# INDA23PlusPlus/isaklm-raytracer

Measured on AMD Instinct MI355X. Metric: Msamples/sec (W×H×spp/s) at 1920×1080; achieved HBM GB/s vs peak, higher is better.
Workload: dtype f32

## Files before the change

### include/isaklm_rt.h

```cpp
#ifndef ISAKLM_RT_H
#define ISAKLM_RT_H

#include <stddef.h>
#include <stdint.h>
#ifndef __cplusplus
#include <stdbool.h>
#endif

#ifdef __cplusplus
extern "C" {
#endif

#define RT_ABI_VERSION 12

typedef struct RtUChar4 { uint8_t x, y, z, w; } RtUChar4;

#ifdef ISAKLM_RT_CALLER_TYPES
#ifndef __cplusplus
#error "ISAKLM_RT_CALLER_TYPES: the reference's types are C++ (anonymous unions, constructors)"
#endif
struct Vec2D;
struct Vec3D;
struct Texture;
struct Material;
// ... 210 lines not shown
    int max_depth;
    int kernel;
    void *stream;
    unsigned long long *counters_device;
    unsigned long long *wave_times_device;
    int wf_tail;
    int wf_finish_waves;
    int profile;
    int wf_descent_cap;
    int wf_postpone;
    int wf_wide;
    int shard_id;
    int num_shards;
    int wf_pipelines;
    int wf_long_depth;
    int traversal;
    int overlap;
    int check_interval;
    int debug;
    int coalesce_passes;
} RtOptions;

#define RT_TRAVERSAL_BOUNDED 0
#define RT_TRAVERSAL_KD 1
#define RT_TRAVERSAL_BOUNDED_COUNTED 2
#define RT_DEBUG_CALL_LOG 1
#define RT_DEBUG_LONG_LOG 2
#define RT_DEBUG_CHECK_FAULT 4
#define RT_DEBUG_LONG_QUIT 8
#define RT_DEBUG_SERIAL_LONG_FIRST 16
#define RT_DEBUG_SERIAL_FIN_FIRST 32
#define RT_DEBUG_WIDE_CAP1 64
#define RT_DEBUG_COUNT_LONG_ONLY 128

typedef struct RtProfile {
    int iterations;
    int trace_launches, shade_launches, finish_launches;
    float start_ms;
    float trace_ms;
    float shade_ms;
    float finish_ms;
    float call_ms;
    float trace_union_ms;
    int pipelines;
} RtProfile;
int rt_last_profile(RtProfile *out);
int rt_profile_history(RtProfile *out, int cap, int *count, int reset);

#define RT_DEV_HIST_BINS 18
typedef struct RtDeviations {
    unsigned long long watchdog_paths;
    unsigned long long cut_paths;
    unsigned long long max_deep_depth;
    unsigned long long deep_paths;
    unsigned long long deep_hist[RT_DEV_HIST_BINS];
    unsigned long long bounded_checked;
    unsigned long long bounded_mismatches;
    float mismatch_ray[6];
    unsigned long long owed_pixels;
    unsigned long long owed_passes;
    unsigned long long long_safety_quits;
    unsigned long long stranded_pixels;
    unsigned long long check_dropped;
    unsigned long long linger_expiries;
    unsigned long long long_closed;
    unsigned long long wide_overflows;
// ... 136 lines not shown
```

### isaklm-raytracer_amd/csrc/bvh_trace.h

```cpp
#pragma once
#include "bvh_common.h"
#include "rt_kernels.h"

namespace rtk {

#if defined(__HIP_DEVICE_COMPILE__)
#define RT_CONST __attribute__((address_space(4)))
#else
#define RT_CONST
#endif
__device__ __forceinline__ RtF4 ldc4(const RtF4 *p)
{
    const RT_CONST RtF4 *q = (const RT_CONST RtF4 *)p;
    return RtF4{q->x, q->y, q->z, q->w};
}
__device__ __forceinline__ uint2 ldc_u2(const void *p)
{
    const RT_CONST uint32_t *q = (const RT_CONST uint32_t *)p;
    return make_uint2(q[0], q[1]);
}
__device__ __forceinline__ float ldc_f(const uint32_t *p) { return __uint_as_float(*(const RT_CONST uint32_t *)p); }
__device__ __forceinline__ uint4 ldc_u4(const uint32_t *p)
{
    const RT_CONST uint4 *q = (const RT_CONST uint4 *)p;
// ... 138 lines not shown
    if (!rt_bvh_box(lx.x, ly.x, lz.x, hx.x, hy.x, hz.x, sl, best, t0)) t0 = INFINITY;
    if (!rt_bvh_box(lx.y, ly.y, lz.y, hx.y, hy.y, hz.y, sl, best, t1)) t1 = INFINITY;
    if (!rt_bvh_box(lx.z, ly.z, lz.z, hx.z, hy.z, hz.z, sl, best, t2)) t2 = INFINITY;
    if (!rt_bvh_box(lx.w, ly.w, lz.w, hx.w, hy.w, hz.w, sl, best, t3)) t3 = INFINITY;
    auto cswap = [](float &ta, uint32_t &ra, float &tb, uint32_t &rb) {
        const bool sw = tb < ta;
        const float t = sw ? tb : ta, u = sw ? ta : tb;
        const uint32_t r = sw ? rb : ra, q = sw ? ra : rb;
        ta = t;
        tb = u;
        ra = r;
        rb = q;
    };
    cswap(t0, r0, t1, r1);
    cswap(t2, r2, t3, r3);
    cswap(t0, r0, t2, r2);
    cswap(t1, r1, t3, r3);
    cswap(t1, r1, t2, r2);
    if (t3 != INFINITY) {
        stk.put(sp, r3, t3);
        ++sp;
    }
    if (t2 != INFINITY) {
        stk.put(sp, r2, t2);
        ++sp;
    }
    if (t1 != INFINITY) {
        stk.put(sp, r1, t1);
        ++sp;
    }
    return t0 != INFINITY ? r0 : RT_BVH_EMPTY;
}

template <bool COUNT, bool PARK, typename STACK>
__device__ __forceinline__ bool bvh4_query(const RtDevScene &sc, Vec3D o, Vec3D d, float best0, STACK &stk, Cnt &cn,
                                           int cap, bool resume, BvhPark &pk)
{
    const RtSlab sl = rt_slab(o, d, rt_ray_margin(o.x, o.y, o.z, sc.bvh_scale));
    int sp = 0;
    uint32_t cur = 0;
    float best = best0;
    int tk = -1;
    if (PARK && resume) {
        sp = pk.sp;
        cur = pk.cur;
        best = pk.best;
        tk = pk.tk;
    }
    int steps = 0;
    while (true) {
        while (!(cur & RT_BVH_LEAF)) {
            if (PARK) {
                if (steps >= cap) {
                    pk.cur = cur;
                    pk.sp = sp;
                    pk.best = best;
                    pk.tk = tk;
                    return false;
                }
                ++steps;
            }
            if (COUNT) cn.v[RT_CNT_B_BVH_NODE]++;
            const uint32_t next = bvh4_children(sc, cur, sl, best, stk, sp);
            cur = next != RT_BVH_EMPTY ? next : bvh_pop(stk, sp, best);
        }
        if (cur == RT_BVH_EMPTY) break;
        const uint32_t first = (cur & ~RT_BVH_LEAF) >> 3, end = first + (cur & 7u) + 1u;
        if (COUNT) cn.v[RT_CNT_B_BVH_TRI] += end - first;
        leaf_scan_min<COUNT>(sc.bvh_a, sc.bvh_bary, first, end, o, d, best, tk, cn);
        cur = bvh_pop(stk, sp, best);
        if (cur == RT_BVH_EMPTY) break;
    }
    pk.best = best;
    pk.tk = tk;
    return true;
}

template <bool COUNT, typename STACK>
__device__ __forceinline__ float bvh4_bound(const RtDevScene &sc, Vec3D o, Vec3D d, float best, STACK &stk, Cnt &cn,
                                            int &tstar, int &tk)
{
    BvhPark pk;
    (void)bvh4_query<COUNT, false>(sc, o, d, best, stk, cn, 0, false, pk);
    tk = pk.tk;
    tstar = pk.tk >= 0 ? (int)sc.bvh_bary[pk.tk].tri : -1;
    return pk.best;
}
template <bool COUNT, typename STACK>
__device__ __forceinline__ float bvh4_bound(const RtDevScene &sc, Vec3D o, Vec3D d, float best, STACK &stk, Cnt &cn,
                                            int &tstar)
{
    int tk;
    return bvh4_bound<COUNT>(sc, o, d, best, stk, cn, tstar, tk);
}

template <bool COUNT>
__device__ __forceinline__ bool kd_certified(const RtDevScene &sc, const Vec3D o, const Vec3D d, const float entry,
                                             const float root_exit, const float s_min, const int tk, int &hit,
                                             float &hbx, float &hby, float &hbz, Cnt &c, const bool count = true)
{
#if RT_KD_CERT
    if (!sc.kd_cert.safe) return false;
    if (rt_kd_cert(sc.kd_cert, o, d, entry, root_exit, s_min, tk) != RT_CERT_OK) return false;
    const RtIsectBary *r = sc.bvh_bary + tk;
    float cx, cy, cz;
    if (!rt_tri_bary(ldc4(&r->b), ldc4(&r->c), ldc4(&r->d), ldc_f(&r->rd), o, d, s_min, cx, cy, cz))
        return false;
    if (COUNT && count) {
        c.v[RT_CNT_HIT]++;
        c.cert[0]++;
    }
    hit = (int)ldc_u2(&r->rd).y;
    hbx = cx;
    hby = cy;
    hbz = cz;
    return true;
// ... 69 lines not shown
        kd_pop(stk, sp, root_exit, node, entry, exit_);
    }
}

template <bool COUNT, typename STACK>
__device__ __forceinline__ int trace_bvh(const RtDevScene &sc, const Vec3D o, const Vec3D d, float &hbx, float &hby,
                                         float &hbz, STACK &stk, Cnt &c)
{
    if (COUNT) c.v[RT_CNT_RAY]++;
    float entry, exit_;
    if (!bbox_hit(sc, o, d, entry, exit_)) return -1;
    const float root_exit = exit_;
    float s_min = -INFINITY;
    int tstar = -1;
    if (rt_bounded_ray(o, d, sc.split_vals, sc.split_off)) {
        int tk = -1;
        s_min = RT_BVH4 ? bvh4_bound<COUNT>(sc, o, d, exit_, stk, c, tstar, tk)
                        : bvh_bound<COUNT>(sc, o, d, exit_, stk, c);
        if (!(s_min < root_exit)) return -1;
        int hit;
        if (kd_certified<COUNT>(sc, o, d, entry, root_exit, s_min, tk, hit, hbx, hby, hbz, c)) return hit;
    }
    float hs;
    const int h = kd_bounded<COUNT>(sc, o, d, entry, root_exit, s_min, tstar, hbx, hby, hbz, hs, stk, c);
    if (COUNT && h >= 0) c.cert[1]++;
    return h;
}

#define RT_PARK_DONE 0
#define RT_PARK_BVH 1
#define RT_PARK_KD 2
template <bool COUNT, typename STACK>
__device__ __forceinline__ int trace_bvh_park(const RtDevScene &sc, const Vec3D o, const Vec3D d, int &hit, float &hbx,
                                              float &hby, float &hbz, STACK &stk, Cnt &c, int cap, int resume,
                                              bool defer_kd, BvhPark &pk)
{
    if (COUNT && resume == RT_PARK_DONE) c.v[RT_CNT_RAY]++;
    hit = -1;
    float entry, exit_;
    if (!bbox_hit(sc, o, d, entry, exit_)) return RT_PARK_DONE;
    const float root_exit = exit_;
    float s_min = -INFINITY;
    int tstar = -1;
    if (rt_bounded_ray(o, d, sc.split_vals, sc.split_off)) {
        if (resume != RT_PARK_KD) {
            if (!bvh4_query<COUNT, true>(sc, o, d, exit_, stk, c, cap, resume == RT_PARK_BVH, pk)) return RT_PARK_BVH;
            if (!(pk.best < root_exit)) return RT_PARK_DONE;
            if (kd_certified<COUNT>(sc, o, d, entry, root_exit, pk.best, pk.tk, hit, hbx, hby, hbz, c))
                return RT_PARK_DONE;
            if (RT_KD_CERT && defer_kd) return RT_PARK_KD;
        }
        s_min = pk.best;
        if (pk.tk >= 0) tstar = (int)sc.bvh_bary[pk.tk].tri;
    }
    float hs;
    hit = kd_bounded<COUNT>(sc, o, d, entry, root_exit, s_min, tstar, hbx, hby, hbz, hs, stk, c);
    if (COUNT && hit >= 0) c.cert[1]++;
    return RT_PARK_DONE;
}

template <typename STACK>
__device__ __forceinline__ int trace_s(const RtDevScene &sc, const Vec3D o, const Vec3D d, float &hs, STACK &stk,
                                       Cnt &c)
{
    float entry, exit_;
    if (!bbox_hit(sc, o, d, entry, exit_)) return -1;
    float bx, by, bz;
    return kd_bounded<false, true>(sc, o, d, entry, exit_, -INFINITY, -1, bx, by, bz, hs, stk, c);
}

template <typename STACK>
__device__ __forceinline__ bool occluded_bvh(const RtDevScene &sc, const Vec3D o, const Vec3D d, const float tmax,
                                             STACK &stk, Cnt &c, bool &early)
{
    early = false;
    float entry, exit_;
    if (!bbox_hit(sc, o, d, entry, exit_)) return false;
    const float root_exit = exit_;
    const float best0 = fminf(root_exit, tmax);
// ... 14 lines not shown
```

### isaklm-raytracer_amd/csrc/host/trace_host.h

```cpp
#pragma once
#include <math.h>
#include <stdint.h>
#include <stdio.h>
#include <stdlib.h>
#include <string.h>

#include <algorithm>
#include <chrono>
#include <utility>
#include <vector>

#include "../bvh_common.h"
#include "bvh_build.h"
#include "rt_host.h"

namespace trace_host {

inline float bitsf(uint32_t u)
{
    float f;
    memcpy(&f, &u, 4);
    return f;
}
inline uint32_t fbits(float f)
// ... 221 lines not shown
            for (int k = 3; k >= 1; --k)
                if (t[k] != INFINITY) stk.push_back(B{r[k], t[k]});
            cur = t[0] != INFINITY ? r[0] : pop();
        }
        if (cur == RT_BVH_EMPTY) break;
        const uint32_t first = (cur & ~RT_BVH_LEAF) >> 3, end = first + (cur & 7u) + 1u;
        obs.bvh_leaf();
        for (uint32_t e = first; e < end; ++e) {
            float s, b[3];
            obs.bvh_test();
            if (!rt_tri_plane(h.bvh_a[e], o, d, INFINITY, s) || !(s <= best)) continue;
            const bool lt = s < best;
            if (!lt && tk < 0) continue;
            const RtIsectBary &R = h.bvh_bary[e];
            if (!rt_tri_bary(R.b, R.c, R.d, bitsf(R.rd), o, d, s, b[0], b[1], b[2])) continue;
            if (lt) {
                best = s;
                tk = (int)e;
            } else {
                tk = TK_TIE;
            }
        }
        cur = pop();
        if (cur == RT_BVH_EMPTY) break;
    }
    return Smin{best, tk};
}
inline Smin bvh4_smin(const rt_host::PreparedHost &h, Vec3D o, Vec3D d, float best)
{
    NoObserver none;
    return bvh4_smin(h, o, d, best, none);
}

template <class Obs>
float bvh_bound(const rt_host::PreparedHost &h, Vec3D o, Vec3D d, float best, Obs &obs)
{
    const RtSlab sl = rt_slab(o, d, rt_ray_margin(o.x, o.y, o.z, h.bvh_scale));
    struct B { uint32_t ref; float tn; };
    B stk[RT_BVH_STACK];
    int sp = 0;
    uint32_t cur = 0;
    while (true) {
        if (!(cur & RT_BVH_LEAF)) {
            obs.bvh_node();
            const RtF4 *nd = &h.bvh_nodes[4 * (size_t)cur];
            const uint32_t c0 = fbits(nd[3].x), c1 = fbits(nd[3].y);
            float tn0, tn1;
            const bool h0 = rt_bvh_box(nd[0].x, nd[0].y, nd[0].z, nd[0].w, nd[1].x, nd[1].y, sl, best, tn0) &&
                            c0 != RT_BVH_EMPTY;
            const bool h1 = rt_bvh_box(nd[1].z, nd[1].w, nd[2].x, nd[2].y, nd[2].z, nd[2].w, sl, best, tn1) &&
                            c1 != RT_BVH_EMPTY;
            if (h0 && h1) {
                const bool sf = tn1 < tn0;
                stk[sp++] = B{sf ? c0 : c1, sf ? tn0 : tn1};
                cur = sf ? c1 : c0;
                continue;
            }
            if (h0 || h1) {
                cur = h0 ? c0 : c1;
                continue;
            }
        } else {
            obs.bvh_leaf();
            const uint32_t first = (cur & ~RT_BVH_LEAF) >> 3, end = first + (cur & 7u) + 1u;
            for (uint32_t e = first; e < end; ++e) {
                float s, b[3];
// ... 288 lines not shown
```

### isaklm-raytracer_amd/csrc/wavefront.hip

```cpp
#include <hip/hip_runtime.h>

#include <stdio.h>
#include <stdlib.h>
#include <string.h>
#include <time.h>

#include <algorithm>
#include <chrono>
#include <atomic>
#include <map>
#include <mutex>
#include <thread>
#include <vector>

#include "bvh_trace.h"
#include "path_event.h"
#include "rt_kernels.h"
#include "rt_launch.h"
#include "rt_workspace.h"
#include "wf_check_grid.h"

using namespace rtk;

#include "wf_state.h"
// ... 443 lines not shown
    const RtDevFrame &fr = c.fr;
    const hipStream_t stream = c.stream;
    const int long_depth = c.long_depth, debug = c.debug;
    const uint32_t check_mask = c.check_mask;
    const size_t slots = (size_t)fr.width * fr.height;
    const bool chain_asked = c.overlap;
    const bool overlap = c.overlap && !fr.reset;
    if (!w.cus) {
        hipDeviceProp_t prop;
        w.cus = hipGetDeviceProperties(&prop, c.dev) == hipSuccess && prop.multiProcessorCount > 0
                    ? prop.multiProcessorCount
                    : 256;
    }
    const int grid = w.cus * 4 * WF_FIN_BVH_WAVES / (WF_BLOCK / 64);
    const ChainKey key = chain_key(c);
    const bool chained = overlap && w.chain_open && !fr.reset && memcmp(&key, &w.key, sizeof key) == 0;
    if (!chained && join_all(w, stream) != 0) return -1;
    if (ensure(w, slots, grid, 1) != 0) return -1;
    Pipe &pp = w.pipe[0];
    WfState st = pp.st;
    whole_state(st, c);
    const int long_return = st.long_return;
    st.fresh_n = (uint32_t)(((fr.width + 15) / 16) * ((fr.height + 15) / 16)) * 256u;
    st.linger = overlap ? 0ull : WF_FIN_LINGER;
    st.chk_mask = check_mask;
    const int par = (int)(w.call_seq & 1);
    unsigned long long chk_want = 0;
    if (ensure_records(w, wf_check_records(slots, (unsigned long long)fr.passes, check_mask,
                                           long_depth > 0 ? long_depth : RT_DEEP_PATH, WF_CHECK_CAP, &chk_want)) != 0)
        return -1;
    st.chk = check_mask == 0xFFFFFFFFu ? nullptr : w.chk + 3 * (size_t)w.chk_cap * (size_t)par;
    st.chk_cap = w.chk_cap;
    st.chk_ctr = w.chk_ctr + par;
    st.chk_fault = (debug & RT_DEBUG_CHECK_FAULT) ? 1 : 0;
    if ((debug & RT_DEBUG_LONG_LOG) && !w.long_log_buf &&
        hipMalloc((void **)&w.long_log_buf, 8 * 4 * 65536) != hipSuccess) {
        w.long_log_buf = nullptr;
        return -1;
    }
    unsigned long long *const long_log_buf = w.long_log_buf;
    st.long_log = (debug & RT_DEBUG_LONG_LOG) ? long_log_buf : nullptr;
    int fgrid = (int)((slots + WF_BLOCK - 1) / WF_BLOCK);
    const int fmax = long_return ? grid - WF_LONG_BLOCKS : grid;
    fgrid = fgrid > fmax ? fmax : fgrid;
    const uint32_t k = (uint32_t)(w.call_seq % 8);
    st.fin_live = long_return ? w.fin_live + k : nullptr;
    st.call_id = (uint32_t)w.call_seq + 1u;
    if (!chained) {
        if (long_return) {
            if (hipMemsetAsync(st.long_ctr, 0, 256, stream) != hipSuccess) return -1;
            if (hipMemsetAsync(st.long_ent, 0, (size_t)st.long_cap * 8, stream) != hipSuccess) return -1;
            if (hipMemsetAsync(st.ret_ring, 0, (size_t)st.long_cap * 8, stream) != hipSuccess) return -1;
            if (hipMemsetAsync(st.ret_ctr, 0, 256, stream) != hipSuccess) return -1;
        }
        if (st.long_log && hipMemsetAsync(long_log_buf, 0, 8 * 4 * 65536, stream) != hipSuccess) return -1;
    }
    ++w.call_seq;
    const hipStream_t s = pp.stream;
    if (hipEventRecord(w.fork, stream) != hipSuccess || hipStreamWaitEvent(s, w.fork, 0) != hipSuccess) return -1;
    if (hipMemsetAsync(st.counts, 0, 256, s) != hipSuccess) return -1;
    if (st.fin_live && hipMemsetD32Async((hipDeviceptr_t)st.fin_live, (int)(fgrid * (WF_BLOCK / 64)), 1, s) != hipSuccess)
        return -1;
    if (st.chk) {
        if (!w.chk_done[par].wait_on(s)) return -1;
        if (hipMemsetAsync(st.chk_ctr, 0, 4, s) != hipSuccess) return -1;
    }
    if (long_return && hipMemsetD32Async((hipDeviceptr_t)st.chain_flag, overlap ? 1 : 0, 1, s) != hipSuccess) return -1;
// ... 496 lines not shown
```

### isaklm-raytracer_amd/csrc/wf_finish_kernels.h

```cpp
#pragma once

namespace {

__device__ __forceinline__ uint32_t ld_sc1(const uint32_t *p)
{
    return __hip_atomic_load(const_cast<uint32_t *>(p), __ATOMIC_RELAXED, __HIP_MEMORY_SCOPE_AGENT);
}

__device__ __forceinline__ void st_sc1(uint32_t *p, uint32_t v)
{
    __hip_atomic_store(p, v, __ATOMIC_RELAXED, __HIP_MEMORY_SCOPE_AGENT);
}

__device__ __forceinline__ bool fresh_pixel(const RtDevFrame &fr, uint32_t e, int &slot)
{
    const uint32_t tiles_x = (uint32_t)(fr.width + 15) / 16u;
    const uint32_t t = e >> 8, w = (e >> 6) & 3u, l = e & 63u;
    const int x = (int)((t % tiles_x) * 16u + (w & 1u) * 8u + (l & 7u));
    const int y = (int)((t / tiles_x) * 16u + (w >> 1) * 8u + (l >> 3));
    if (x >= fr.width || y >= fr.height || !rt_row_owned(fr, y)) return false;
    slot = y * fr.width + x;
    return true;
}

// ... 25 lines not shown
    Cnt c;
    if (COUNT) c.zero();
    const uint32_t n_heavy = st.fresh && st.heavy_list ? *st.heavy_n : 0u;
    const uint32_t n = st.fresh ? n_heavy + st.fresh_n : st.counts[6 + q];
    const int limit = fr.max_depth > 0 ? fr.max_depth : RT_WATCHDOG_BOUNCES;
    const int lane = __lane_id();
    if (lane == 0) {
        unsigned long long *const ret_word = reinterpret_cast<unsigned long long *>(st.ret_ctr);
        if (st.fin_live && !(__hip_atomic_load(st.fin_live, __ATOMIC_RELAXED, __HIP_MEMORY_SCOPE_AGENT) & WF_FIN_STARTED))
            __hip_atomic_fetch_or(st.fin_live, WF_FIN_STARTED, __ATOMIC_RELAXED, __HIP_MEMORY_SCOPE_AGENT);
        if (st.long_return)
            __hip_atomic_fetch_add(ret_word, 1ull << 32, __ATOMIC_RELAXED, __HIP_MEMORY_SCOPE_AGENT);
        if (st.span) atomicMin(st.span, __builtin_amdgcn_s_memrealtime());
        if (st.long_log && blockIdx.x == 0 && threadIdx.x == 0) st.long_log[0] = __builtin_amdgcn_s_memrealtime();
    }
#if WF_NEE_LDS
    __shared__ float s_nee[10 * WF_BLOCK];
    PathRegsL p;
    p.rp.w = s_nee + wbase;
    p.cont.w = s_nee + 3 * WF_BLOCK + wbase;
    p.snorm.w = s_nee + 6 * WF_BLOCK + wbase;
    p.light.w = reinterpret_cast<int *>(s_nee + 9 * WF_BLOCK) + wbase;
#else
    PathRegs p;
#endif
    p.slot = 0;
    p.ro = p.rd = rt_v3(0, 0, 0);
    bool active = false, exhausted = false;
    bool rel = false;
    unsigned long long idle_since = 0;
    uint32_t quiet_trips = 0;
    uint32_t idle_trips = 0;
    bool seated = false;
#if WF_BVH_PARK
    __shared__ uint32_t s_pk_cur[WF_BLOCK];
    __shared__ int s_pk_sp[WF_BLOCK];
    __shared__ float s_pk_best[WF_BLOCK];
    __shared__ int s_pk_tk[WF_BLOCK];
    int parked = RT_PARK_DONE;
#endif
    while (true) {
        while (st.fresh && __any(rel)) {
            if (rel) {
                WfCold &cs = WF_COLD(st);
                uint32_t x = RT_PX_BUSY;
                if (__hip_atomic_compare_exchange_strong(cs.pxo + p.slot, &x, 0u, __ATOMIC_RELAXED, __ATOMIC_RELAXED,
                                                         __HIP_MEMORY_SCOPE_AGENT)) {
                    rel = false;
                } else {
                    x = __hip_atomic_exchange(cs.pxo + p.slot, RT_PX_BUSY, __ATOMIC_RELAXED, __HIP_MEMORY_SCOPE_AGENT);
                    const uint32_t owed = x & RT_PX_PASSES;
                    __hip_atomic_fetch_max(cs.ret_ctr + 5, owed, __ATOMIC_RELAXED, __HIP_MEMORY_SCOPE_AGENT);
                    __hip_atomic_fetch_add(cs.ret_ctr + 6, 1u, __ATOMIC_RELAXED, __HIP_MEMORY_SCOPE_AGENT);
                    const RtDevFrame cf = WF_COLD_FRAME(fr);
                    atomicAdd(cf.dev_stats + RT_DEV_OWED_PIXELS, 1ull);
                    atomicAdd(cf.dev_stats + RT_DEV_OWED_PASSES, (unsigned long long)owed);
                    p.passes_left = (int)owed;
                    const Vec3D fb = cf.fb[p.slot];
                    const float sq = cf.sq[p.slot];
                    const int count = cf.count[p.slot];
                    if (start_sample<COUNT>(cf, WF_COLD_CAM(cam), (int)p.slot, p.passes_left, p.rng, fb, sq, count, p.ro, p.rd,
                                            c)) {
                        begin_path(p);
                        rel = false;
                        active = true;
                    }
                }
            }
        }
        if (st.long_return) {
            const bool chained = st.linger == 0ull;
            const bool idle = !active && !(chained && exhausted);
            const unsigned long long im = __ballot(idle);
// ... 152 lines not shown
                if (idle_since == 0) idle_since = __builtin_amdgcn_s_memrealtime();
                if (__hip_atomic_load(cs.long_ctr + 3, __ATOMIC_RELAXED, __HIP_MEMORY_SCOPE_AGENT) == 0u)
                    ++quiet_trips;
                else
                    quiet_trips = 0;
                ++idle_trips;
                bool out = quiet_trips < WF_FIN_QUIET_TRIPS && idle_trips < WF_FIN_LINGER_TRIPS &&
                           __hip_atomic_load(cs.ret_ctr + 3, __ATOMIC_RELAXED, __HIP_MEMORY_SCOPE_AGENT) != 0u;
                if (out && !seated) {
                    if (__hip_atomic_fetch_add(cs.ret_ctr + 4, 1u, __ATOMIC_RELAXED, __HIP_MEMORY_SCOPE_AGENT) <
                        WF_FIN_LINGER_WAVES)
                        seated = true;
                    else
                        out = false;
                }
                unsigned long long w = __hip_atomic_load(ret_word, __ATOMIC_RELAXED, __HIP_MEMORY_SCOPE_AGENT);
                const uint32_t cl = __hip_atomic_load(ret_claimed, __ATOMIC_RELAXED, __HIP_MEMORY_SCOPE_AGENT);
                if ((uint32_t)w == cl &&
                    (!out || __builtin_amdgcn_s_memrealtime() - idle_since > st.linger) &&
                    __hip_atomic_compare_exchange_strong(ret_word, &w, w - (1ull << 32), __ATOMIC_RELAXED,
                                                         __ATOMIC_RELAXED, __HIP_MEMORY_SCOPE_AGENT)) {
                    leave = 1;
                    if (out) atomicAdd(WF_COLD_FRAME(fr).dev_stats + RT_DEV_LINGER_EXP, 1ull);
                }
            }
            if (__shfl(leave, 0)) break;
            __builtin_amdgcn_s_sleep(8);
            continue;
        }
        idle_since = 0;
        quiet_trips = 0;
        idle_trips = 0;
        bool to_long = false;
#if WF_BVH_PARK && RT_KD_CERT
        const unsigned long long kd_pend = __ballot(active && parked == RT_PARK_KD);
        const bool run_kd = kd_pend != 0ull && (__popcll(kd_pend) >= WF_KD_PEND_MIN ||
                                                __ballot(active && parked != RT_PARK_KD) == 0ull);
        if (active && (parked != RT_PARK_KD || run_kd)) {
#else
        if (active) {
#endif
            float bx = 0.0f, by = 0.0f, bz = 0.0f;
#if WF_BVH_PARK
            int hit;
            BvhPark pk{0u, 0, 0.0f, -1};
            if (parked != RT_PARK_DONE) pk = BvhPark{s_pk_cur[tid], s_pk_sp[tid], s_pk_best[tid], s_pk_tk[tid]};
            parked = trace_bvh_park<COUNT>(sc, p.ro, p.rd, hit, bx, by, bz, stk, c, WF_BVH_PARK, parked, true, pk);
            const bool done = parked == RT_PARK_DONE;
            if (!done) {
                s_pk_cur[tid] = pk.cur;
                s_pk_sp[tid] = pk.sp;
                s_pk_best[tid] = pk.best;
                s_pk_tk[tid] = pk.tk;
            }
#else
            const int hit = trace_bvh<COUNT>(sc, p.ro, p.rd, bx, by, bz, stk, c);
            const bool done = true;
#endif
            if (!COUNT && st.chk && done) {
                uint32_t h = p.slot * 0x9E3779B1u ^ (uint32_t)p.passes_left * 0x85EBCA77u ^
                             (uint32_t)p.depth * 0xC2B2AE3Du ^ (p.shadow ? 0x27D4EB2Fu : 0u);
                h ^= h >> 15;
                h *= 0x2C1B3C6Du;
                h ^= h >> 12;
                const bool rec = (h & st.chk_mask) == 0u;
                if (__any(rec)) {
                    WfCold &cs = WF_COLD(st);
                    const uint32_t i = wave_append(cs.chk_ctr, rec);
                    if (rec && i < cs.chk_cap) {
                        cs.chk[3 * (size_t)i] =
                            RtF4{p.ro.x, p.ro.y, p.ro.z, __int_as_float(cs.chk_fault ? (hit >= 0 ? hit ^ 1 : 0) : hit)};
                        cs.chk[3 * (size_t)i + 1] = RtF4{p.rd.x, p.rd.y, p.rd.z, bx};
                        cs.chk[3 * (size_t)i + 2] = RtF4{by, bz, 0.0f, 0.0f};
                    }
                }
            }
            if (done) {
                const RtDevFrame cf = WF_COLD_FRAME(fr);
                const bool want = shade_step<COUNT>(sc, cf, WF_COLD_CAM(cam), p, hit, bx, by, bz, limit, c);
                to_long = want && st.long_depth > 0 && p.depth > st.long_depth;
                if (!want || to_long) store_regs(WF_COLD(st), cf, p);
                if (!want) {
                    active = false;
                    rel = st.fresh != 0;
                }
            }
        }
        if (__any(to_long)) {
            WfCold &cs = WF_COLD(st);
            if (publish_long_capped(cs, to_long, p.slot, p.ro, p.rd) && to_long) {
                active = false;
                if (cs.heavy) {
                    const uint8_t h = cs.heavy[p.slot];
                    if (h < 255) cs.heavy[p.slot] = (uint8_t)(h + 1);
                }
            }
        }
    }
    if (COUNT) {
        flush_counters(c, fr.counters);
        flush_cert_counters(c, fr.dev_stats);
    }
    WfCold &ce = WF_COLD(st);
    if (ce.span && lane == 0) atomicMax(ce.span + 1, __builtin_amdgcn_s_memrealtime());
// ... 192 lines not shown
```

### isaklm-raytracer_amd/csrc/wf_state.h

```cpp
#pragma once

#define WF_BLOCK 256
#ifndef WF_TBLOCK
#define WF_TBLOCK 256
#endif
static_assert(WF_BLOCK % WF_TBLOCK == 0 && WF_TBLOCK % 64 == 0, "WF_TBLOCK must divide WF_BLOCK in whole waves");
#ifndef WF_SHADE_PRIO
#define WF_SHADE_PRIO 3
#endif
#ifndef WF_SHADE_WAVES
#define WF_SHADE_WAVES 6
#endif
#ifndef WF_LONG_WAVES
#define WF_LONG_WAVES 4
#endif
#ifndef WF_LONG_PRIO
#define WF_LONG_PRIO 3
#endif
#ifndef WF_FIN_LINGER
#define WF_FIN_LINGER 100000000ull
#endif
#ifndef WF_FIN_LINGER_WAVES
#define WF_FIN_LINGER_WAVES 256u
#endif
#ifndef WF_HEAVY_FIRST
#define WF_HEAVY_FIRST 1
#endif
#define WF_HEAVY_BLOCKS 256
#ifndef WF_HEAVY_SPLIT
#define WF_HEAVY_SPLIT 4
#endif
#ifndef WF_FIN_QUIET_TRIPS
#define WF_FIN_QUIET_TRIPS 4096u
#endif
#define WF_FIN_LINGER_TRIPS 1000000u
#ifndef WF_FIN_OCC
#define WF_FIN_OCC 1
#endif
#ifndef WF_TAIL_PRIO
#define WF_TAIL_PRIO 2
#endif
#ifndef WF_LDS_STACK
#define WF_LDS_STACK 8
#endif
#ifndef WF_TRACE_WAVES
#define WF_TRACE_WAVES 6
#endif
#ifndef WF_BVH_LDS
#define WF_BVH_LDS 10
#endif
#ifndef WF_CHECK_BLOCKS
#define WF_CHECK_BLOCKS 256
#endif
#ifndef WF_BVH_PARK
#define WF_BVH_PARK 6
#endif
#ifndef WF_KD_PEND_MIN
#define WF_KD_PEND_MIN 4
#endif
#ifndef WF_FIN_BVH_WAVES
#define WF_FIN_BVH_WAVES 4
#endif
#ifndef WF_NEE_LDS
#define WF_NEE_LDS 1
#endif
#ifndef WF_FIN_SMALL_WAVES
#define WF_FIN_SMALL_WAVES 3
#endif
#define WF_SPILL_ENTRIES \
    ((RT_STACK_DEPTH - WF_LDS_STACK) > (RT_BVH_STACK - WF_BVH_LDS) ? (RT_STACK_DEPTH - WF_LDS_STACK) \
                                                                    : (RT_BVH_STACK - WF_BVH_LDS))
#define WF_TAIL_DEFAULT 65536u
#define WF_FINISH_WAVES_DEFAULT 2048u
#define WF_FINISH_WAVES_SMALL 512u
#define WF_DESCENT_CAP_DEFAULT 5
#define WF_POSTPONE_DEFAULT 20
#define WF_TIMELINE_LAUNCHES 4096
#define WF_WIDE_TAIL_LANES 32
#define WF_FIN_WIDE_MIN_ENTRIES (1 << 18)
#define WF_MAX_PIPES 6
#define WF_PIPES_DEFAULT 3
#ifndef WF_LONG_DEPTH_DEFAULT
#define WF_LONG_DEPTH_DEFAULT 64
#endif
#define WF_LONG_DEPTH_MIN 16
#define WF_COALESCE_DEFAULT 256
#ifndef WF_LONG_BLOCKS
#define WF_LONG_BLOCKS 64
#endif
// ... 187 lines not shown
```

### isaklm-raytracer_amd/rt.py

```python
import ctypes
import os

import numpy as np

HERE = os.path.dirname(os.path.abspath(__file__))
LIB_PATH = os.path.join(HERE, "libisaklm_rt.so")
LIB_PATH = os.environ.get("ISAKLM_RT_LIB_OVERRIDE", LIB_PATH)


class Vec3D(ctypes.Structure):
    _fields_ = [("x", ctypes.c_float), ("y", ctypes.c_float), ("z", ctypes.c_float)]


class Bounding_Box(ctypes.Structure):
    _fields_ = [("min", Vec3D), ("max", Vec3D)]


class KD_Tree(ctypes.Structure):
    _fields_ = [("bounding_box", Bounding_Box), ("nodes", ctypes.c_void_p), ("triangle_indicies", ctypes.c_void_p)]


class Scene(ctypes.Structure):
    _fields_ = [("triangles", ctypes.c_void_p), ("triangle_count", ctypes.c_int),
                ("light_indicies", ctypes.c_void_p), ("light_count", ctypes.c_int), ("kd_tree", KD_Tree)]
# ... 106 lines not shown
HANDOFF_FIELDS = ("owed_pixels", "owed_passes", "long_safety_quits", "stranded_pixels", "check_dropped",
                  "linger_expiries", "long_closed", "wide_overflows")


def deviation_stats(reset=False):
    d = RtDeviations()
    check(lib().rt_deviation_stats(ctypes.byref(d), int(reset)))
    out = {"watchdog_paths": d.watchdog_paths, "cut_paths": d.cut_paths, "max_deep_depth": d.max_deep_depth,
           "deep_paths": d.deep_paths, "deep_hist": [int(v) for v in d.deep_hist],
           "bounded_checked": int(d.bounded_checked), "bounded_mismatches": int(d.bounded_mismatches),
           "mismatch_ray": [float(v) for v in d.mismatch_ray]}
    out.update({k: int(getattr(d, k)) for k in HANDOFF_FIELDS})
    return out


def kd_cert_stats(reset=False):
    if not hasattr(lib(), "rt_kd_cert_stats"):
        raise RtError(f"{LIB_PATH} was built before rt_kd_cert_stats was added (within ABI {ABI_VERSION}): rebuild it")
    a, b = ctypes.c_ulonglong(0), ctypes.c_ulonglong(0)
    check(lib().rt_kd_cert_stats(ctypes.byref(a), ctypes.byref(b), int(reset)))
    return int(a.value), int(b.value)


def join(stream=None):
    check(lib().rt_join(stream))


ABI_VERSION = 12
E_INCOMPLETE = -7
DEBUG_CALL_LOG, DEBUG_LONG_LOG, DEBUG_CHECK_FAULT, DEBUG_LONG_QUIT = 1, 2, 4, 8
DEBUG_SERIAL_LONG_FIRST, DEBUG_SERIAL_FIN_FIRST = 16, 32
DEBUG_COUNT_LONG_ONLY = 128
DEBUG_WIDE_CAP1 = 64
TRIANGLE_BYTES = 152
NODE_BYTES = 20
COUNTER_NAMES = ["node", "tri", "hit", "texel", "nee", "sample", "skip", "ray", "watchdog", "maxdepth"]
FINISH_COUNTER_NAMES = ["finish_node", "finish_tri", "finish_ray", "cand", "plane", "deep_push", "t_descend", "t_leaves",
                        "t_fetch", "rounds", "chunks", "bary", "wide_calls", "wide_rounds", "t_wide", "t_wide_load", "t_wide_leaf", "t_wide_expand",
                       "t_leaf_wait", "t_leaf_setup", "t_leaf_test", "t_leaf_bary", "spill_push", "spill_pop",
                        "pend_lanes", "leaf_tests", "t_desc_wait", "b_bvh_node", "b_bvh_tri", "b_bary"]
N_COUNTERS = 40

_lib = None


class RtError(RuntimeError):
    pass


def lib():
    global _lib
    if _lib is None:
        if not os.path.exists(LIB_PATH):
            raise RtError(f"{LIB_PATH} is missing: run __graft_entry__.build() (no CPU fallback exists)")
        L = ctypes.CDLL(LIB_PATH)
        vp, i, sz = ctypes.c_void_p, ctypes.c_int, ctypes.c_size_t
        L.rt_last_error.restype = ctypes.c_char_p
        L.rt_version.restype = ctypes.c_char_p
        L.rt_device_alloc.argtypes = [ctypes.POINTER(vp), sz]
        L.rt_free.argtypes = [vp]
        L.rt_upload.argtypes = [vp, vp, sz]
        L.rt_download.argtypes = [vp, vp, sz]
        L.rt_memset.argtypes = [vp, i, sz]
        L.rt_device_count.argtypes = [ctypes.POINTER(i)]
        L.rt_set_device.argtypes = [i]
        L.rt_host_free.argtypes = [vp]
# ... 932 lines not shown
```

Measured before the change: 930.4.

## Replace per-lane BVH park cap with wave-coherent node/leaf phase budget

The BVH4 traversal in the finish kernel no longer parks each lane after a fixed count of node steps. It now runs a wavefront-wide loop that ballots which lanes sit at internal nodes versus leaves and picks a node or leaf phase each iteration, aiming to cut divergence between box tests and triangle scans. Each call is capped by a total body budget of 14 before the ray is parked. A host-side simulator of both schedules and a debug flag that forces a budget of 1 are also added. The extra ballots per iteration and the changed park granularity could raise overhead or the number of parked trips.

```diff
diff --git a/include/isaklm_rt.h b/include/isaklm_rt.h
--- a/include/isaklm_rt.h
+++ b/include/isaklm_rt.h
@@ -266,6 +266,7 @@
 #define RT_DEBUG_SERIAL_FIN_FIRST 32
 #define RT_DEBUG_WIDE_CAP1 64
 #define RT_DEBUG_COUNT_LONG_ONLY 128
+#define RT_DEBUG_BUDGET1 256
 
 typedef struct RtProfile {
     int iterations;
diff --git a/isaklm-raytracer_amd/csrc/bvh_trace.h b/isaklm-raytracer_amd/csrc/bvh_trace.h
--- a/isaklm-raytracer_amd/csrc/bvh_trace.h
+++ b/isaklm-raytracer_amd/csrc/bvh_trace.h
@@ -194,34 +194,17 @@
     return t0 != INFINITY ? r0 : RT_BVH_EMPTY;
 }
 
-template <bool COUNT, bool PARK, typename STACK>
-__device__ __forceinline__ bool bvh4_query(const RtDevScene &sc, Vec3D o, Vec3D d, float best0, STACK &stk, Cnt &cn,
-                                           int cap, bool resume, BvhPark &pk)
+template <bool COUNT, typename STACK>
+__device__ __forceinline__ void bvh4_query(const RtDevScene &sc, Vec3D o, Vec3D d, float best0, STACK &stk, Cnt &cn,
+                                           BvhPark &pk)
 {
     const RtSlab sl = rt_slab(o, d, rt_ray_margin(o.x, o.y, o.z, sc.bvh_scale));
     int sp = 0;
     uint32_t cur = 0;
     float best = best0;
     int tk = -1;
-    if (PARK && resume) {
-        sp = pk.sp;
-        cur = pk.cur;
-        best = pk.best;
-        tk = pk.tk;
-    }
-    int steps = 0;
     while (true) {
         while (!(cur & RT_BVH_LEAF)) {
-            if (PARK) {
-                if (steps >= cap) {
-                    pk.cur = cur;
-                    pk.sp = sp;
-                    pk.best = best;
-                    pk.tk = tk;
-                    return false;
-                }
-                ++steps;
-            }
             if (COUNT) cn.v[RT_CNT_B_BVH_NODE]++;
             const uint32_t next = bvh4_children(sc, cur, sl, best, stk, sp);
             cur = next != RT_BVH_EMPTY ? next : bvh_pop(stk, sp, best);
@@ -235,7 +218,61 @@
     }
     pk.best = best;
     pk.tk = tk;
-    return true;
+}
+
+template <bool COUNT, typename STACK>
+__device__ __forceinline__ bool bvh4_query_budget(const RtDevScene &sc, Vec3D o, Vec3D d, float best0, STACK &stk,
+                                                  Cnt &cn, const int budget, bool resume, BvhPark &pk)
+{
+    const RtSlab sl = rt_slab(o, d, rt_ray_margin(o.x, o.y, o.z, sc.bvh_scale));
+    int sp = 0;
+    uint32_t cur = 0;
+    float best = best0;
+    int tk = -1;
+    if (resume) {
+        sp = pk.sp;
+        cur = pk.cur;
+        best = pk.best;
+        tk = pk.tk;
+    }
+    auto leaf_visit = [&]() {
+        const uint32_t first = (cur & ~RT_BVH_LEAF) >> 3, end = first + (cur & 7u) + 1u;
+        if (COUNT) cn.v[RT_CNT_B_BVH_TRI] += end - first;
+        leaf_scan_min<COUNT>(sc.bvh_a, sc.bvh_bary, first, end, o, d, best, tk, cn);
+        cur = bvh_pop(stk, sp, best);
+    };
+    int bodies = 0;
+    bool lead = __any((cur & RT_BVH_LEAF) != 0u) != 0;
+    bool owed = __any(!(cur & RT_BVH_LEAF)) != 0;
+    while (true) {
+        const bool node = !(cur & RT_BVH_LEAF), leaf = !node && cur != RT_BVH_EMPTY;
+        const unsigned long long nm = __ballot(node), lm = __ballot(leaf);
+        if (!(nm | lm)) break;
+        bool leaf_phase;
+        if (lead) {
+            leaf_phase = true;
+            lead = false;
+        } else if (owed) {
+            leaf_phase = false;
+            owed = false;
+        } else {
+            if (bodies >= budget) break;
+            leaf_phase = __popcll(lm) > __popcll(nm);
+        }
+        if (leaf_phase) {
+            if (leaf) leaf_visit();
+        } else if (node) {
+            if (COUNT) cn.v[RT_CNT_B_BVH_NODE]++;
+            const uint32_t next = bvh4_children(sc, cur, sl, best, stk, sp);
+            cur = next != RT_BVH_EMPTY ? next : bvh_pop(stk, sp, best);
+        }
+        ++bodies;
+    }
+    pk.cur = cur;
+    pk.sp = sp;
+    pk.best = best;
+    pk.tk = tk;
+    return cur == RT_BVH_EMPTY;
 }
 
 template <bool COUNT, typename STACK>
@@ -243,7 +280,7 @@
                                             int &tstar, int &tk)
 {
     BvhPark pk;
-    (void)bvh4_query<COUNT, false>(sc, o, d, best, stk, cn, 0, false, pk);
+    bvh4_query<COUNT>(sc, o, d, best, stk, cn, pk);
     tk = pk.tk;
     tstar = pk.tk >= 0 ? (int)sc.bvh_bary[pk.tk].tri : -1;
     return pk.best;
@@ -379,7 +416,7 @@
 #define RT_PARK_KD 2
 template <bool COUNT, typename STACK>
 __device__ __forceinline__ int trace_bvh_park(const RtDevScene &sc, const Vec3D o, const Vec3D d, int &hit, float &hbx,
-                                              float &hby, float &hbz, STACK &stk, Cnt &c, int cap, int resume,
+                                              float &hby, float &hbz, STACK &stk, Cnt &c, int budget, int resume,
                                               bool defer_kd, BvhPark &pk)
 {
     if (COUNT && resume == RT_PARK_DONE) c.v[RT_CNT_RAY]++;
@@ -391,7 +428,7 @@
     int tstar = -1;
     if (rt_bounded_ray(o, d, sc.split_vals, sc.split_off)) {
         if (resume != RT_PARK_KD) {
-            if (!bvh4_query<COUNT, true>(sc, o, d, exit_, stk, c, cap, resume == RT_PARK_BVH, pk)) return RT_PARK_BVH;
+            if (!bvh4_query_budget<COUNT>(sc, o, d, exit_, stk, c, budget, resume == RT_PARK_BVH, pk)) return RT_PARK_BVH;
             if (!(pk.best < root_exit)) return RT_PARK_DONE;
             if (kd_certified<COUNT>(sc, o, d, entry, root_exit, pk.best, pk.tk, hit, hbx, hby, hbz, c))
                 return RT_PARK_DONE;
diff --git a/isaklm-raytracer_amd/csrc/host/trace_host.h b/isaklm-raytracer_amd/csrc/host/trace_host.h
--- a/isaklm-raytracer_amd/csrc/host/trace_host.h
+++ b/isaklm-raytracer_amd/csrc/host/trace_host.h
@@ -277,6 +277,191 @@
     return bvh4_smin(h, o, d, best, none);
 }
 
+struct Bvh4Walk {
+    const rt_host::PreparedHost *h = nullptr;
+    Vec3D o, d;
+    RtSlab sl;
+    struct B { uint32_t ref; float tn; };
+    std::vector<B> stk;
+    uint32_t cur = RT_BVH_EMPTY;
+    float best = 0.0f;
+    int tk = -1;
+    long long bodies = 0, trips = 0;
+
+    void start(const rt_host::PreparedHost &hh, Vec3D oo, Vec3D dd, float best0)
+    {
+        h = &hh;
+        o = oo;
+        d = dd;
+        sl = rt_slab(o, d, rt_ray_margin(o.x, o.y, o.z, hh.bvh_scale));
+        stk.clear();
+        cur = 0;
+        best = best0;
+        tk = -1;
+        bodies = trips = 0;
+    }
+    bool done() const { return cur == RT_BVH_EMPTY; }
+    bool at_node() const { return !(cur & RT_BVH_LEAF); }
+    bool at_leaf() const { return (cur & RT_BVH_LEAF) && cur != RT_BVH_EMPTY; }
+    int leaf_chunks() const { return (int)((cur & 7u) + 1u + 3u) / 4; }
+    uint32_t pop()
+    {
+        while (!stk.empty()) {
+            const B e = stk.back();
+            stk.pop_back();
+            if (e.tn <= best) return e.ref;
+        }
+        return RT_BVH_EMPTY;
+    }
+    void node_step()
+    {
+        ++bodies;
+        const float *f = reinterpret_cast<const float *>(&h->bvh4[8 * (size_t)cur]);
+        const uint32_t *rf = reinterpret_cast<const uint32_t *>(f + 24);
+        float t[4];
+        uint32_t r[4];
+        for (int k = 0; k < 4; ++k) {
+            r[k] = rf[k];
+            if (!rt_bvh_box(f[k], f[4 + k], f[8 + k], f[12 + k], f[16 + k], f[20 + k], sl, best, t[k])) t[k] = INFINITY;
+        }
+        auto cswap = [&](int a, int b) {
+            if (t[b] < t[a]) {
+                std::swap(t[a], t[b]);
+                std::swap(r[a], r[b]);
+            }
+        };
+        cswap(0, 1);
+        cswap(2, 3);
+        cswap(0, 2);
+        cswap(1, 3);
+        cswap(1, 2);
+        for (int k = 3; k >= 1; --k)
+            if (t[k] != INFINITY) stk.push_back(B{r[k], t[k]});
+        cur = t[0] != INFINITY ? r[0] : pop();
+    }
+    void leaf_visit()
+    {
+        ++bodies;
+        const uint32_t first = (cur & ~RT_BVH_LEAF) >> 3, end = first + (cur & 7u) + 1u;
+        for (uint32_t e = first; e < end; ++e) {
+            float s, b[3];
+            if (!rt_tri_plane(h->bvh_a[e], o, d, INFINITY, s) || !(s <= best)) continue;
+            const bool lt = s < best;
+            if (!lt && tk < 0) continue;
+            const RtIsectBary &R = h->bvh_bary[e];
+            if (!rt_tri_bary(R.b, R.c, R.d, bitsf(R.rd), o, d, s, b[0], b[1], b[2])) continue;
+            if (lt) {
+                best = s;
+                tk = (int)e;
+            } else {
+                tk = TK_TIE;
+            }
+        }
+        cur = pop();
+    }
+};
+
+struct WaveTrip {
+    long long node_bodies = 0, leaf_bodies = 0, leaf_chunks = 0, lane_bodies = 0, lanes = 0, finished = 0;
+};
+
+inline WaveTrip wave_call_budget(std::vector<Bvh4Walk *> &q, int budget)
+{
+    WaveTrip w;
+    auto count = [&](auto pred) {
+        int n = 0;
+        for (Bvh4Walk *l : q) n += pred(*l) ? 1 : 0;
+        return n;
+    };
+    for (Bvh4Walk *l : q) {
+        ++l->trips;
+        ++w.lanes;
+    }
+    long long bodies = 0;
+    bool lead = count([](const Bvh4Walk &l) { return l.at_leaf(); }) > 0;
+    bool owed = count([](const Bvh4Walk &l) { return l.at_node(); }) > 0;
+    while (true) {
+        const int nn = count([](const Bvh4Walk &l) { return l.at_node(); });
+        const int nl = count([](const Bvh4Walk &l) { return l.at_leaf(); });
+        if (nn + nl == 0) break;
+        bool leaf_phase;
+        if (lead) {
+            leaf_phase = true;
+            lead = false;
+        } else if (owed) {
+            leaf_phase = false;
+            owed = false;
+        } else {
+            if (bodies >= budget) break;
+            leaf_phase = nl > nn;
+        }
+        if (leaf_phase) {
+            int chunks = 0;
+            for (Bvh4Walk *l : q)
+                if (l->at_leaf()) {
+                    chunks = std::max(chunks, l->leaf_chunks());
+                    l->leaf_visit();
+                    ++w.lane_bodies;
+                }
+            ++w.leaf_bodies;
+            w.leaf_chunks += chunks;
+        } else {
+            for (Bvh4Walk *l : q)
+                if (l->at_node()) {
+                    l->node_step();
+                    ++w.lane_bodies;
+                }
+            ++w.node_bodies;
+        }
+        ++bodies;
+    }
+    for (Bvh4Walk *l : q) w.finished += l->done();
+    return w;
+}
+
+inline WaveTrip wave_call_lane_cap(std::vector<Bvh4Walk *> &q, int cap)
+{
+    WaveTrip w;
+    std::vector<int> steps(q.size(), 0);
+    std::vector<char> parked(q.size(), 0);
+    for (Bvh4Walk *l : q) {
+        ++l->trips;
+        ++w.lanes;
+    }
+    while (true) {
+        while (true) {
+            bool ran = false;
+            for (size_t i = 0; i < q.size(); ++i) {
+                if (parked[i] || !q[i]->at_node()) continue;
+                if (steps[i] >= cap) {
+                    parked[i] = 1;
+                    continue;
+                }
+                ++steps[i];
+                q[i]->node_step();
+                ++w.lane_bodies;
+                ran = true;
+            }
+            if (!ran) break;
+            ++w.node_bodies;
+        }
+        int chunks = 0;
+        bool leaf = false;
+        for (size_t i = 0; i < q.size(); ++i) {
+            if (parked[i] || !q[i]->at_leaf()) continue;
+            chunks = std::max(chunks, q[i]->leaf_chunks());
+            q[i]->leaf_visit();
+            ++w.lane_bodies;
+            leaf = true;
+        }
+        if (!leaf) break;
+        ++w.leaf_bodies;
+        w.leaf_chunks += chunks;
+    }
+    for (Bvh4Walk *l : q) w.finished += l->done();
+    return w;
+}
+
 template <class Obs>
 float bvh_bound(const rt_host::PreparedHost &h, Vec3D o, Vec3D d, float best, Obs &obs)
 {
diff --git a/isaklm-raytracer_amd/csrc/wavefront.hip b/isaklm-raytracer_amd/csrc/wavefront.hip
--- a/isaklm-raytracer_amd/csrc/wavefront.hip
+++ b/isaklm-raytracer_amd/csrc/wavefront.hip
@@ -499,7 +499,7 @@
     st.chk = check_mask == 0xFFFFFFFFu ? nullptr : w.chk + 3 * (size_t)w.chk_cap * (size_t)par;
     st.chk_cap = w.chk_cap;
     st.chk_ctr = w.chk_ctr + par;
-    st.chk_fault = (debug & RT_DEBUG_CHECK_FAULT) ? 1 : 0;
+    st.chk_fault = ((debug & RT_DEBUG_CHECK_FAULT) ? 1 : 0) | ((debug & RT_DEBUG_BUDGET1) ? WF_DEBUG_BUDGET1 : 0);
     if ((debug & RT_DEBUG_LONG_LOG) && !w.long_log_buf &&
         hipMalloc((void **)&w.long_log_buf, 8 * 4 * 65536) != hipSuccess) {
         w.long_log_buf = nullptr;
diff --git a/isaklm-raytracer_amd/csrc/wf_finish_kernels.h b/isaklm-raytracer_amd/csrc/wf_finish_kernels.h
--- a/isaklm-raytracer_amd/csrc/wf_finish_kernels.h
+++ b/isaklm-raytracer_amd/csrc/wf_finish_kernels.h
@@ -81,13 +81,11 @@
     uint32_t quiet_trips = 0;
     uint32_t idle_trips = 0;
     bool seated = false;
-#if WF_BVH_PARK
     __shared__ uint32_t s_pk_cur[WF_BLOCK];
     __shared__ int s_pk_sp[WF_BLOCK];
     __shared__ float s_pk_best[WF_BLOCK];
     __shared__ int s_pk_tk[WF_BLOCK];
     int parked = RT_PARK_DONE;
-#endif
     while (true) {
         while (st.fresh && __any(rel)) {
             if (rel) {
@@ -306,7 +304,7 @@
         quiet_trips = 0;
         idle_trips = 0;
         bool to_long = false;
-#if WF_BVH_PARK && RT_KD_CERT
+#if RT_KD_CERT
         const unsigned long long kd_pend = __ballot(active && parked == RT_PARK_KD);
         const bool run_kd = kd_pend != 0ull && (__popcll(kd_pend) >= WF_KD_PEND_MIN ||
                                                 __ballot(active && parked != RT_PARK_KD) == 0ull);
@@ -315,11 +313,11 @@
         if (active) {
 #endif
             float bx = 0.0f, by = 0.0f, bz = 0.0f;
-#if WF_BVH_PARK
             int hit;
             BvhPark pk{0u, 0, 0.0f, -1};
             if (parked != RT_PARK_DONE) pk = BvhPark{s_pk_cur[tid], s_pk_sp[tid], s_pk_best[tid], s_pk_tk[tid]};
-            parked = trace_bvh_park<COUNT>(sc, p.ro, p.rd, hit, bx, by, bz, stk, c, WF_BVH_PARK, parked, true, pk);
+            const int budget = COUNT && (WF_COLD(st).chk_fault & WF_DEBUG_BUDGET1) ? 1 : WF_BVH_BUDGET;
+            parked = trace_bvh_park<COUNT>(sc, p.ro, p.rd, hit, bx, by, bz, stk, c, budget, parked, true, pk);
             const bool done = parked == RT_PARK_DONE;
             if (!done) {
                 s_pk_cur[tid] = pk.cur;
@@ -327,10 +325,6 @@
                 s_pk_best[tid] = pk.best;
                 s_pk_tk[tid] = pk.tk;
             }
-#else
-            const int hit = trace_bvh<COUNT>(sc, p.ro, p.rd, bx, by, bz, stk, c);
-            const bool done = true;
-#endif
             if (!COUNT && st.chk && done) {
                 uint32_t h = p.slot * 0x9E3779B1u ^ (uint32_t)p.passes_left * 0x85EBCA77u ^
                              (uint32_t)p.depth * 0xC2B2AE3Du ^ (p.shadow ? 0x27D4EB2Fu : 0u);
@@ -343,7 +337,7 @@
                     const uint32_t i = wave_append(cs.chk_ctr, rec);
                     if (rec && i < cs.chk_cap) {
                         cs.chk[3 * (size_t)i] =
-                            RtF4{p.ro.x, p.ro.y, p.ro.z, __int_as_float(cs.chk_fault ? (hit >= 0 ? hit ^ 1 : 0) : hit)};
+                            RtF4{p.ro.x, p.ro.y, p.ro.z, __int_as_float((cs.chk_fault & 1) ? (hit >= 0 ? hit ^ 1 : 0) : hit)};
                         cs.chk[3 * (size_t)i + 1] = RtF4{p.rd.x, p.rd.y, p.rd.z, bx};
                         cs.chk[3 * (size_t)i + 2] = RtF4{by, bz, 0.0f, 0.0f};
                     }
diff --git a/isaklm-raytracer_amd/csrc/wf_state.h b/isaklm-raytracer_amd/csrc/wf_state.h
--- a/isaklm-raytracer_amd/csrc/wf_state.h
+++ b/isaklm-raytracer_amd/csrc/wf_state.h
@@ -52,9 +52,10 @@
 #ifndef WF_CHECK_BLOCKS
 #define WF_CHECK_BLOCKS 256
 #endif
-#ifndef WF_BVH_PARK
-#define WF_BVH_PARK 6
-#endif
+#ifndef WF_BVH_BUDGET
+#define WF_BVH_BUDGET 14
+#endif
+#define WF_DEBUG_BUDGET1 2
 #ifndef WF_KD_PEND_MIN
 #define WF_KD_PEND_MIN 4
 #endif
diff --git a/isaklm-raytracer_amd/rt.py b/isaklm-raytracer_amd/rt.py
--- a/isaklm-raytracer_amd/rt.py
+++ b/isaklm-raytracer_amd/rt.py
@@ -162,6 +162,7 @@
 DEBUG_SERIAL_LONG_FIRST, DEBUG_SERIAL_FIN_FIRST = 16, 32
 DEBUG_COUNT_LONG_ONLY = 128
 DEBUG_WIDE_CAP1 = 64
+DEBUG_BUDGET1 = 256
 TRIANGLE_BYTES = 152
 NODE_BYTES = 20
 COUNTER_NAMES = ["node", "tri", "hit", "texel", "nee", "sample", "skip", "ray", "watchdog", "maxdepth"]
```

Result: faster. 1049 (median of 6 runs) (+12.7%).
